# ShamG1/marl-traffic-intersection

Measured on AMD Instinct MI355X. Metric: agent-steps/sec (whole node) at 4096 envs × 8 agents × 64-beam lidar; 1/2/4/8 GPU, higher is better.
Workload: dtype f32

## Files before the change

marl-traffic-intersection_amd/csrc/mev_kernels.hip:

```cpp
#include <type_traits>

#include <cfloat>
#include <cstdlib>

#include "mev_kernels.h"
#include "mev_world.h"
#include "mev_nsort.h"

namespace mev {

#ifdef MEV_STAMPS
#define STAMP_RAW(k)                                                     \
    do {                                                                 \
        __builtin_amdgcn_wave_barrier();                                 \
        if (threadIdx.x == 0) p.debug[e * 8 + (k)] = __builtin_amdgcn_s_memtime(); \
    } while (0)
#if defined(MEV_STAMPS_R)
#undef STAMP_RAW
#define STAMP_RAW(k)                                                     \
    do {                                                                 \
        __builtin_amdgcn_wave_barrier();                                 \
        if (threadIdx.x == 0) p.debug[e * 8 + (k)] = __builtin_amdgcn_s_memrealtime(); \
    } while (0)
#ifndef MEV_STAMPS_POSTEND
#define MEV_STAMPS_POSTEND 0
#endif
#define STAMP(k) do { if ((k) == 0) STAMP_RAW(1); if ((k) == (MEV_STAMPS_POSTEND ? 6 : 5)) STAMP_RAW(2); } while (0)
#else
#define STAMP(k) STAMP_RAW(k)
#endif
#elif defined(MEV_STAMPS_Q)
__shared__ unsigned long long mev_qst[8 * 8];
#define QSTAMP(k) do { if ((threadIdx.x & 63) == 0) mev_qst[(threadIdx.x >> 6) * 8 + (k)] = __builtin_amdgcn_s_memtime(); } while (0)
#define STAMP(k) do { if ((k) == 0) QSTAMP(1); if ((k) == 1) QSTAMP(2); if ((k) == 2) QSTAMP(3); \
                      if ((k) == 5) QSTAMP(4); if ((k) == 6) QSTAMP(6); } while (0)
#else
#define STAMP(k) do {} while (0)
#endif
#ifndef QSTAMP
#define QSTAMP(k) do {} while (0)
// ... 2352 lines not shown
                const size_t g = (size_t)z * en + (size_t)e * N + tid;
                if (a.rows.reward) gmem(a.rows.reward)[g] = 0.0f;
                if (a.rows.done) gmem(a.rows.done)[g] = 0;
                if (a.rows.status) gmem(a.rows.status)[g] = 0;
                if constexpr (SAMPLE) {
                    if (sc.in->actions_out) (void)sample_action(sc, N, e, tid, z, true);
                }
            }
        }
        if constexpr (EVAL) {
            if (bad) {
                const EvalOuts& ev = a.ev;
                if (tid < N && ev.returns) gmem(ev.returns)[(size_t)e * N + tid] = 0.0f;
                if (tid == 0) {
                    if (ev.substeps) gmem(ev.substeps)[e] = 0;
                    if (ev.term) gmem(ev.term)[e] = 0;
                    if (ev.trunc) gmem(ev.trunc)[e] = 0;
                }
                if constexpr (LEAF) {
                    const Outputs& out = a.out;
                    const int ls = a.p.lidar_slots;
                    if (tid < N) gmem(a.lf.alive)[(size_t)(e - a.lf.c0) * N + tid] = 0;
                    for (int i = 0; i < N; ++i) {
                        float* row = out.obs + ((size_t)e * N + i) * out.obs_ld;
                        for (int cc = tid; cc < out.obs_ld - ls; cc += WAVE) row[cc < OBS_HEAD ? cc : cc + ls] = 0.0f;
                    }
                }
            }
        }
    }
}


template <class T>
__device__ __forceinline__ T lidar_keep(T v) {
    asm volatile("" : "+v"(v));
    return v;
}
__device__ __forceinline__ int safe_steps(float safe, float stp, float inv_stp) {
    const int j = lidar_keep((int)(safe * inv_stp));
    return (safe >= stp) ? j : 0;
}

__device__ inline float road_safe(float fx, float fy, float dx, float dy, float idx, float idy, float iadx,
                                  float iady, float rwm, float ccen, float crf) {
    const float big = 1.0e6f;
    const float rx = fx - 375.0f, ry = fy - 375.0f;
    const float ax = fabs_f(rx), ay = fabs_f(ry);
    const float sx = ax < rwm ? rwm * iadx - rx * idx : 0.0f;
    const float sy = ay < rwm ? rwm * iady - ry * idy : 0.0f;
    const float sqm = ccen - 1.55f, rg = crf + 2.0f;
    const float qx = rx != 0.0f ? rx : dx, qy = ry != 0.0f ? ry : dy;
    const float ocx = rx - (qx >= 0.0f ? ccen : -ccen), ocy = ry - (qy >= 0.0f ? ccen : -ccen);
    const float bq = ocx * dx + ocy * dy;
    const float cq = ocx * ocx + ocy * ocy - rg * rg;
    const float disc = bq * bq - cq;
    const float troot = lidar_keep(-bq - __builtin_amdgcn_sqrtf(disc));
    const float tdisc = cq <= 0.0f ? 0.0f : ((disc < 0.0f || bq >= 0.0f) ? big : troot);
    const float tsq = fminf(sqm * iadx - rx * idx, sqm * iady - ry * idy);
    const float tq = fminf(rx * dx < 0.0f ? -rx * idx : big, ry * dy < 0.0f ? -ry * idy : big);
    const float sc = fmaxf(ax, ay) < sqm ? fminf(tdisc, fminf(tsq, tq)) : 0.0f;
    const float road = fmaxf(fmaxf(sx, sy), sc);
    const float tx = (dx > 0.0f ? 748.5f - fx : fx - 0.5f) * iadx;
    const float ty = (dy > 0.0f ? 748.5f - fy : fy - 0.5f) * iady;
    return fminf(road, fminf(tx, ty));
}

__device__ inline float road_safe_uniform(float fx, float fy, float dx, float dy, float idx, float idy, float iadx,
                                          float iady, float rwm, float ccen, float crf) {
    const float big = 1.0e6f;
    const float rx = fx - 375.0f, ry = fy - 375.0f;
    const float ax = fabs_f(rx), ay = fabs_f(ry);
    const float sqm = ccen - 1.55f, rg = crf + 2.0f;
    float road = 0.0f;
    if (__builtin_amdgcn_readfirstlane((int)(ax < rwm))) road = fmaxf(road, rwm * iadx - rx * idx);
    if (__builtin_amdgcn_readfirstlane((int)(ay < rwm))) road = fmaxf(road, rwm * iady - ry * idy);
    if (__builtin_amdgcn_readfirstlane((int)(fmaxf(ax, ay) < sqm))) {
        const float qx = rx != 0.0f ? rx : dx, qy = ry != 0.0f ? ry : dy;
        const float ocx = rx - (qx >= 0.0f ? ccen : -ccen), ocy = ry - (qy >= 0.0f ? ccen : -ccen);
        const float bq = ocx * dx + ocy * dy;
        const float cq = ocx * ocx + ocy * ocy - rg * rg;
        const float disc = bq * bq - cq;
        const float troot = lidar_keep(-bq - __builtin_amdgcn_sqrtf(disc));
        const float tdisc = cq <= 0.0f ? 0.0f : ((disc < 0.0f || bq >= 0.0f) ? big : troot);
        const float tsq = fminf(sqm * iadx - rx * idx, sqm * iady - ry * idy);
        const float tq = fminf(rx * dx < 0.0f ? -rx * idx : big, ry * dy < 0.0f ? -ry * idy : big);
        road = fmaxf(road, fminf(tdisc, fminf(tsq, tq)));
    }
    const float tx = (dx > 0.0f ? 748.5f - fx : fx - 0.5f) * iadx;
    const float ty = (dy > 0.0f ? 748.5f - fy : fy - 0.5f) * iady;
    return fminf(road, fminf(tx, ty));
}

__device__ inline float atan2_fast(float y, float x) {
    const float ax = fabs_f(x), ay = fabs_f(y);
    const float mx = fmaxf(ax, ay), mn = fminf(ax, ay);
    const float t = mn * __builtin_amdgcn_rcpf(fmaxf(mx, 1e-30f));
    const float s2 = t * t;
    float r = ((-0.0464964749f * s2 + 0.15931422f) * s2 - 0.327622764f) * s2 * t + t;
    r = ay > ax ? 1.57079637f - r : r;
    r = x < 0.0f ? 3.14159274f - r : r;
    return y < 0.0f ? -r : r;
}

__device__ inline float wrap_pi_fast(float a) { return a - 6.28318531f * rintf(a * 0.159154943f); }

__device__ inline float box_lo(int lo) { return (float)(lo > 0 ? lo : lo - 1) - 0.01f; }
__device__ inline float box_hi(int hi) { return (float)hi + 1.01f; }

__device__ inline void slab_clip(float c0, float dc, float idc, float a, float b, float& lo, float& hi) {
    if (fabs_f(dc) < 1e-6f) {
        if (c0 < a || c0 > b) { lo = 1.0f; hi = 0.0f; }
        return;
    }
    const float t1 = (a - c0) * idc, t2 = (b - c0) * idc;
    lo = fmaxf(lo, fminf(t1, t2));
    hi = fminf(hi, fmaxf(t1, t2));
}




#ifndef MEV_LIDAR_NPR
#define MEV_LIDAR_NPR 2
#endif
constexpr int LIDAR_NPR = MEV_LIDAR_NPR;
constexpr int kMarchHelp = 16;
constexpr int kNptHelp = 3;
static_assert(kMarchHelp <= 32, "helper groups have at least 2 lanes");

int lidar_group(int R) {
    int g = 256 / (R > 0 ? R : 1);
    return g < 1 ? 1 : (g > 64 ? 64 : g);
}

struct LidarSrcHbm {
    static constexpr bool kBoxLds = false;
    const SimParams& p;
    __device__ float rel(int b) const { return gmem(p.rel_angles)[b]; }
    __device__ bool alive(int g) const { return gmem(p.ego.alive)[g] != 0; }
    __device__ float4 pose(int g) const { return make_float4(egof(p, EF_X)[g], egof(p, EF_Y)[g], egof(p, EF_H)[g], __int_as_float(g)); }
    __device__ void cand(int g, unsigned long long& c0, unsigned long long& c1) const {
        c0 = gmem(p.ob_cand)[2 * g];
        c1 = gmem(p.ob_cand)[2 * g + 1];
    }
    __device__ int4 box(int g, int o) const { return p.ob_box[(size_t)(g / p.N) * p.ob_stride + o]; }
};
struct LidarSrcLds {
    static constexpr bool kBoxLds = true;
    const CarsLDS& el;
    int g0;
    __device__ float rel(int b) const { return el.rel[b]; }
    __device__ bool alive(int g) const { return el.alive[g - g0] != 0; }
    __device__ float4 pose(int g) const {
        const int i = g - g0;
        return make_float4(el.x[i], el.y[i], el.h[i], __int_as_float(g));
    }
    __device__ void cand(int g, unsigned long long& c0, unsigned long long& c1) const {
        c0 = el.cand[2 * (g - g0)];
// ... 5 lines not shown
struct LidarSrcLdsEnvs {
    static constexpr bool kBoxLds = true;
    const CarsLDS& el0;
    int reg;
    const float* relp;
    int env[ENVS];
    __device__ int off(int g) const {
        int j = 0;
#pragma unroll
        for (int u = 1; u < ENVS; ++u) j = g == env[u] ? u : j;
        return j * reg;
    }
    template <class T>
    __device__ const T* at(const T* p0, int g) const {
        return reinterpret_cast<const T*>(reinterpret_cast<const unsigned char*>(p0) + off(g));
    }
    __device__ float rel(int b) const { return relp[b]; }
    __device__ bool alive(int g) const { return at(el0.alive, g)[0] != 0; }
    __device__ float4 pose(int g) const {
        return make_float4(at(el0.x, g)[0], at(el0.y, g)[0], at(el0.h, g)[0], __int_as_float(g));
    }
    __device__ void cand(int g, unsigned long long& c0, unsigned long long& c1) const {
        const unsigned long long* c = at(el0.cand, g);
        c0 = c[0];
        c1 = c[1];
    }
    __device__ int4 box(int g, int o) const { return at(el0.box, g)[o]; }
};

#ifndef MEV_DENSE_ILP
#define MEV_DENSE_ILP 2
#endif
template <bool TAB, int ILP, class Src, int NPT = LIDAR_NPR, bool HELP = false, int PART = 0, int P1 = 0,
          bool WC = false, bool SEGL = false>
__device__ __forceinline__ void lidar_body(const SimParams& p, const Outputs& out, const Src& src, const int G,
                                           const int a0, const int na, const int lane, unsigned char* base,
                                           const LidarLayout& lay, const unsigned long long redo = 0ull,
                                           const unsigned long long alive_in = 0ull) {
    static_assert(!WC || (!TAB && P1 >= WAVE), "the reference's world: no distance table, the beams at compile time");
    using W = StepWorld<WC>;
    using RW = StepRows<WC, P1>;
    const int R = P1 >= WAVE ? P1 : p.R;
    const int LS = P1 >= WAVE ? P1 : p.lidar_slots;
    float4* ag = reinterpret_cast<float4*>(base + lay.ag);
    float2* dir = reinterpret_cast<float2*>(base + lay.dir);
    int* res = reinterpret_cast<int*>(base + lay.res);
#if defined(MEV_STAMPS_R)
    const int se_ = a0 / p.N, sp_ = ((a0 % p.N) / G) & 1;
    if (lane == 0) p.debug[se_ * 8 + 3 + sp_] = __builtin_amdgcn_s_memrealtime();
#endif

    bool alv = false;
    if (PART != 0) alv = (alive_in >> lane) & 1ull;
    else if (lane < na) alv = src.alive(a0 + lane);
    const unsigned long long am = PART != 0 ? alive_in : ballot(alv);
    const int nal = __popcll(am);
    if (PART == 0 && alv) {
        const int g = a0 + lane;
        ag[lane_rank(am)] = src.pose(g);
    }
    if (PART != 2 && __popcll(am) != na) {
        for (int j = 0; j < na; ++j) {
            if ((am >> j) & 1ull) continue;
            if (RW::lidar_u8(out)) {
                uint8_t* crow = RW::lidar_u8(out) + (size_t)(a0 + j) * LS;
                for (int b = lane; b < LS; b += WAVE) crow[b] = (uint8_t)kLidarCodeDead;
                continue;
// ... 29 lines not shown
    auto probes_n = [&](auto np, float cx_, float cy_, float dx_, float dy_, int k_, float& fx, float& fy) -> int {
        int r = -1;
#pragma unroll
        for (int t = 0; t < decltype(np)::value; ++t) {
            const int c = probe(cx_, cy_, dx_, dy_, k_ + t, fx, fy);
            r = r >= 0 ? r : c;
        }
        return r;
    };
    auto probes = [&](float cx_, float cy_, float dx_, float dy_, int k_, float& fx, float& fy) -> int {
        return probes_n(std::integral_constant<int, LIDAR_NPR>{}, cx_, cy_, dx_, dy_, k_, fx, fy);
    };

    unsigned short* queue = reinterpret_cast<unsigned short*>(base + lay.queue);
    int qn = 0;
    const float rel_c0 = lane < R ? src.rel(lane) : 0.0f;
    const float rel_c1 = lane + WAVE < R ? src.rel(lane + WAVE) : 0.0f;
    auto setup = [&](const float4& a, float rel_b, auto small, float2& d, bool uni) -> int {
        float sn, cs;
#if defined(MEV_EXP_FASTSIN)
        sn = __sinf(a.z + rel_b);
        cs = __cosf(a.z + rel_b);
        (void)small;
#else
        if constexpr (decltype(small)::value) sincosf_below120(a.z + rel_b, &sn, &cs);
        else sincosf(a.z + rel_b, &sn, &cs);
#endif
        const float dx = cs, dy = -sn;
        d = make_float2(dx, dy);
        const int px = (int)a.x, py = (int)a.y;
        const unsigned pmax = (unsigned)px > (unsigned)py ? (unsigned)px : (unsigned)py;
        const float idx = __builtin_amdgcn_rcpf(dx), idy = __builtin_amdgcn_rcpf(dy);
        float safe;
        if (uni)
            safe = road_safe_uniform(a.x, a.y, dx, dy, idx, idy, fabs_f(idx), fabs_f(idy), rwm, ccen, crf);
        else
            safe = road_safe(a.x, a.y, dx, dy, idx, idy, fabs_f(idx), fabs_f(idy), rwm, ccen, crf);
        const int k1 = pmax < (unsigned)WIDTH ? 1 + safe_steps(safe, stp, inv_stp) : 0;
        float fx, fy;
        const int r = probes_n(std::integral_constant<int, LIDAR_NPR>{}, a.x, a.y, dx, dy, k1, fx, fy);
        return r >= 0 ? r : -(k1 + LIDAR_NPR) - 1;
    };
    auto pass1_one = [&](auto small, const int j) {
        const float4 a = ag[j];
        for (int b0 = 0; b0 < R; b0 += WAVE) {
            const int b = b0 + lane;
            const bool vb = b < R;
            const float rel_b = b0 == 0 ? rel_c0 : (b0 == WAVE ? rel_c1 : (vb ? src.rel(b) : 0.0f));
            float2 d;
            const int r = setup(a, rel_b, small, d, true);
            if (vb) {
                dir[j * R + b] = d;
                res[j * R + b] = r >= 0 ? r : -r - 1;
            }
            const bool pend = vb && r < 0;
            const unsigned long long m = ballot(pend);
            if (pend) queue[qn + lane_rank(m)] = (unsigned short)(j * R + b);
            qn += __popcll(m);
        }
    };
    const bool dense = P1 >= WAVE ? (P1 & (WAVE - 1)) != 0 : (P1 == 2 || (P1 == 0 && (R & (WAVE - 1)) != 0 && nal > 1));
    auto phase1 = [&](auto small) {
        if constexpr (PART == 2) {
            for (unsigned long long tm = redo; tm; tm &= tm - 1ull) pass1_one(small, __builtin_ctzll(tm));
        } else if (dense) {
            const float invRp = 1.0f / (float)R;
            const int nq = nal * R;
// ... 48 lines not shown
                    if (vb && in) {
                        dir[(j + u) * R + b] = d[u];
                        res[(j + u) * R + b] = r[u] >= 0 ? r[u] : -r[u] - 1;
                    }
                    const bool pend = vb && in && r[u] < 0;
                    const unsigned long long m = ballot(pend);
                    if (pend) queue[qn + lane_rank(m)] = (unsigned short)((j + u) * R + b);
                    qn += __popcll(m);
                }
            }
        }
        }
    };
    const bool hsmall = ballot(lane < nal && !(fabs_f(ag[lane < nal ? lane : 0].z) < 100.0f)) == 0ull;
    if (ILP > 1 && hsmall) phase1(std::true_type{});
    else phase1(std::false_type{});
    wave_lds_sync();
#if defined(MEV_EXP_STOP) && MEV_EXP_STOP == 2
    if (Src::kBoxLds) return;
#endif
#if defined(MEV_STAMPS_R)
    if (lane == 0 && na == p.N) p.debug[se_ * 8 + 4] = __builtin_amdgcn_s_memrealtime();
#endif

    if (PART == 0) __builtin_amdgcn_s_setprio(kPrioP2);
#if defined(MEV_EXP_TSNOMARCH)
    if constexpr (PART == 1) return;
#endif
    const float invR = 1.0f / (float)R;
    int next = qn < WAVE ? qn : WAVE;
    int slot = lane < qn ? (int)queue[lane] : -1;
    float cx = 0.0f, cy = 0.0f, dx = 0.0f, dy = 0.0f, idx = 0.0f, idy = 0.0f, iadx = 0.0f, iady = 0.0f;
    int k = 0;
    auto load_beam = [&](int qq) {
        const int j = (int)(((float)qq + 0.5f) * invR);
        const float4 a = ag[j];
        const float2 d = dir[qq];
        cx = a.x; cy = a.y; dx = d.x; dy = d.y;
        idx = __builtin_amdgcn_rcpf(dx);
        idy = __builtin_amdgcn_rcpf(dy);
        iadx = fabs_f(idx);
        iady = fabs_f(idy);
        k = res[qq];
    };
    if (slot >= 0) load_beam(slot);
    int* hscr = reinterpret_cast<int*>(base + lay.scr);
    bool help = false;
    while (ballot(slot >= 0) != 0ull) {
        if (HELP && next >= qn && __popcll(ballot(slot >= 0)) <= kMarchHelp) {
            help = true;
            break;
        }
        const bool act = slot >= 0;
        float fx, fy;
        int r, npr = LIDAR_NPR;
        if (NPT != LIDAR_NPR && next >= qn) {
            r = probes_n(std::integral_constant<int, NPT>{}, cx, cy, dx, dy, k, fx, fy);
            npr = NPT;
        } else {
            r = probes(cx, cy, dx, dy, k, fx, fy);
        }
        const float safe = road_safe(fx, fy, dx, dy, idx, idy, iadx, iady, rwm, ccen, crf);
        const int kn = k + npr + safe_steps(safe, stp, inv_stp);
        const bool fin = act & ((r >= 0) | (kn >= S));
        if (fin) res[slot] = r >= 0 ? r : (S << 1);
        k = kn;
        const unsigned long long fm = ballot(fin);
        if (fm != 0ull) {
            if (fin) {
                const int nq = next + lane_rank(fm);
                slot = nq < qn ? (int)queue[nq] : -1;
                if (slot >= 0) load_beam(slot);
            }
            next += __popcll(fm);
        }
    }
    if (HELP && help) {
        constexpr int NPH = kNptHelp;
        const unsigned long long am = ballot(slot >= 0);
        const int nb = __popcll(am);
        if (slot >= 0) {
            const int rk = lane_rank(am);
            hscr[2 * rk] = slot;
            hscr[2 * rk + 1] = k;
        }
        wave_lds_sync();
        auto group_march = [&](auto gs_c) {
            constexpr int GS = decltype(gs_c)::value;
            const int gi = lane / GS, j = lane & (GS - 1);
            slot = gi < nb ? hscr[2 * gi] : -1;
            const int k_h = gi < nb ? hscr[2 * gi + 1] : 0;
            if (slot >= 0) load_beam(slot);
            k = k_h;
            while (ballot(slot >= 0) != 0ull) {
                float fx, fy;
                const int k0 = k + j * NPH;
                int r = probes_n(std::integral_constant<int, NPH>{}, cx, cy, dx, dy, k0, fx, fy);
                r = r >= 0 ? r : 0x7fffffff;
                const float safe = road_safe(fx, fy, dx, dy, idx, idy, iadx, iady, rwm, ccen, crf);
                int kn = k0 + NPH + safe_steps(safe, stp, inv_stp);
                r = min(r, __builtin_amdgcn_mov_dpp(r, 0xB1, 0xf, 0xf, false));
                if constexpr (GS == 2) {
                    kn = __builtin_amdgcn_mov_dpp(kn, 0xF5, 0xf, 0xf, false);
                } else {
                    r = min(r, __builtin_amdgcn_mov_dpp(r, 0x4E, 0xf, 0xf, false));
                    kn = __builtin_amdgcn_mov_dpp(kn, 0xFF, 0xf, 0xf, false);
                    if constexpr (GS == 8) {
                        r = min(r, __builtin_amdgcn_mov_dpp(r, 0x141, 0xf, 0xf, false));
                        const int km = __builtin_amdgcn_mov_dpp(kn, 0x141, 0xf, 0xf, false);
                        kn = j < 4 ? km : kn;
                    }
                }
                const bool fin = slot >= 0 && (r != 0x7fffffff || kn >= S);
                if (fin && j == 0) res[slot] = r != 0x7fffffff ? r : (S << 1);
                slot = fin ? -1 : slot;
                k = kn;
            }
        };
        if (nb <= 8) group_march(std::integral_constant<int, 8>{});
        else if (nb <= 16) group_march(std::integral_constant<int, 4>{});
        else group_march(std::integral_constant<int, 2>{});
    }
    wave_lds_sync();
    if constexpr (PART == 1) return;
#if defined(MEV_EXP_STOP) && MEV_EXP_STOP == 3
    if (Src::kBoxLds) return;
#endif
#if defined(MEV_STAMPS_R)
    if (lane == 0 && na == p.N) p.debug[se_ * 8 + 6] = __builtin_amdgcn_s_memrealtime();
#endif

    __builtin_amdgcn_s_setprio(kPrioP3);
    int* seg_jo = reinterpret_cast<int*>(base + lay.seg_jo);
    int4* seg_rg = reinterpret_cast<int4*>(base + lay.seg_rg);
    int4* seg_bx = reinterpret_cast<int4*>(base + lay.seg_bx);
    int* scr = reinterpret_cast<int*>(base + lay.scr);
    int M = 0;
#if defined(MEV_SEG_COUNTS)
    int dbg_t = 0, dbg_pass = 0;
#endif
    if constexpr (!SEGL) {
    unsigned long long cl0 = 0ull, cl1 = 0ull;
    if (lane < nal) src.cand(__float_as_int(ag[lane].w), cl0, cl1);
    for (int j = 0; j < nal; ++j) {
        const unsigned long long c0 = readlane64(cl0, j), c1 = readlane64(cl1, j);
        const int n0 = __popcll(c0);
        if ((c0 >> lane) & 1ull) seg_jo[M + lane_rank(c0)] = (j << 8) | lane;
        if ((c1 >> lane) & 1ull) seg_jo[M + n0 + lane_rank(c1)] = (j << 8) | (lane + WAVE);
        M += n0 + __popcll(c1);
    }
    wave_lds_sync();
    }
    const float rel0 = src.rel(0);
    const bool all_beams = R == 1 || !W::beam_cull(p);
    const float dphi = R > 1 ? (src.rel(R - 1) - rel0) / (float)(R - 1) : 1.0f;
// ... 261 lines not shown
            int rr[8];
#pragma unroll
            for (int u = 0; u < 8; ++u) rr[u] = (j0 + u < nal && beam) ? res[(j0 + u) * R + lane] : 0;
#pragma unroll
            for (int u = 0; u < 8; ++u) {
                if (j0 + u < nal && beam) {
                    const int g = __builtin_amdgcn_readlane(gl, j0 + u);
                    obs_store<true>(&out.obs[(size_t)g * RW::obs_ld(out) + OBS_HEAD + lane], row_value(rr[u]));
                }
            }
        }
    } else {
        for (int j = 0; j < nal; ++j) {
            const int g = __float_as_int(ag[j].w);
            float* row = out.obs + (size_t)g * RW::obs_ld(out) + OBS_HEAD;
            for (int b = lane; b < LS; b += WAVE)
                obs_store<true>(row + b, ((res[j * R + b] & 1) ? march_dist<TAB, WC>(p, res[j * R + b] >> 1) : W::lidar_max(p)) *
                                             W::lidar_inv(p));
        }
    }
}

template <bool TAB>
__global__ __launch_bounds__(256, 8) void k_lidar(SimParams p, Outputs out, int G, int a_begin, int a_end) {
    extern __shared__ __align__(16) unsigned char lds_raw[];
    const int lane = threadIdx.x & (WAVE - 1);
    const int wv = threadIdx.x / WAVE;
    const int blk = xcd_env((int)blockIdx.x, (int)gridDim.x);
    const int a0 = __builtin_amdgcn_readfirstlane(a_begin + (blk * (int)(blockDim.x / WAVE) + wv) * G);
    if (a0 >= a_end) return;
    const int na = a_end - a0 < G ? a_end - a0 : G;
    __builtin_amdgcn_s_setprio(kPrioLidar);
    const LidarLayout lay = lidar_layout(G, p.R, lidar_cand_max(p));
    lidar_body<TAB, 1>(p, out, LidarSrcHbm{p}, G, a0, na, lane, lds_raw + (size_t)wv * (size_t)lay.bytes, lay);
}


template <int NM, int KM>
__host__ __device__ inline StepLayout step_layout_t(const SimParams& p) {
    if constexpr (NM == 0) return step_layout(p);
    else return StepLayout{FixedLayout<NM, KM>::rel, FixedLayout<NM, KM>::rel, FixedLayout<NM, KM>::envw,
                           FixedLayout<NM, KM>::lidar, FixedLayout<NM, KM>::bytes};
}
#ifndef MEV_PHASE1_ILP
#define MEV_PHASE1_ILP 2
#endif
#ifndef MEV_ESPLIT_ILP
#define MEV_ESPLIT_ILP 1
#endif
constexpr int kPhase1Ilp = MEV_PHASE1_ILP;
constexpr int kEsplitIlp = MEV_ESPLIT_ILP;

template <bool TRAFFIC>
__device__ __forceinline__ void deal_append(const SimParams& p, const StepInputs& in, const CarsCtx& cx, const int e) {
    if constexpr (TRAFFIC) {
        if (!(in.deal & 2)) return;
        const int lane0 = threadIdx.x & (WAVE - 1);
        const int x = (int)blockIdx.x & (kDealLists - 1);
        const int nxt = in.deal_ring == 2 ? 0 : in.deal_ring + 1;
        if (lane0 == 0) {
            const int c = (in.auto_reset && cx.ended) ? 0 : (cx.ncnt < kDealClasses - 1 ? cx.ncnt : kDealClasses - 1);
            const int slot = atomicAdd(p.deal_cnt + (size_t)nxt * kDealRingInts + (x * kDealClasses + c) * kDealPad, 1);
            const size_t ring_off = (size_t)nxt * kDealLists * kDealClasses * (size_t)p.E;
            gmem(p.deal_order)[ring_off + ((size_t)x * kDealClasses + c) * p.E + slot] = e;
        }
        if (blockIdx.x == 0 && lane0 < kDealLists * kDealClasses) {
            const int clr = nxt == 2 ? 0 : nxt + 1;
// ... 650 lines not shown
```

marl-traffic-intersection_amd/csrc/mev_step_body.inc:

```
    static_assert(!SPLIT || !TRAFFIC || ESPLIT, "split waves with traffic: the early split");
    static_assert(!WC || (!TRAFFIC && !TAB && NM > 0 && PK == 1 && !SPLIT && P1 >= WAVE && NC > 0),
                  "the world at compile time: one wave per env, the counts at compile time, no table");
    const SimParams& p = *pp;
    extern __shared__ __align__(16) unsigned char step_lds[];
    const int wv = SPLIT ? __builtin_amdgcn_readfirstlane((int)(threadIdx.x >> 6)) : 0;
    int npc_cls = kDealClasses - 1;
    const int e = (TRAFFIC && (in.deal & 1)) ? deal_env(p, in.deal_ring, (int)blockIdx.x, 1, 0, &npc_cls)
                                             : xcd_env((int)blockIdx.x, (int)gridDim.x) * PK;
#if defined(MEV_STAMPS_R)
    STAMP_RAW(0);
#endif
    QSTAMP(0);
    constexpr int KF = TRAFFIC ? KM : 0;
    constexpr bool SEGL = NM == 8 && KF == 0;
    constexpr int NCE = NM == 1 ? 1 : NC;
    const StepLayout sl = step_layout_t<NM, KF>(p);
    constexpr bool DIMS = NM == 0;
    using NLT = NpcLDST<KM, DIMS>;
    CarsLDS el = NM ? carve_cars_lds(step_lds, NM, KF) : carve_cars_lds(step_lds, p.N, cars_k(p), DIMS);
    el.head = reinterpret_cast<float*>(step_lds + sl.head);
    el.rel = reinterpret_cast<float*>(step_lds + sl.rel);
    el.envw = reinterpret_cast<int32_t*>(step_lds + sl.envw);
    if constexpr (!TRAFFIC && NM > 0) {
        static_assert(NM == 0 || FixedLayout<(NM ? NM : 1), 0>::lay.bytes >= kWinBytes, "LDS path windows");
// ... 33 lines not shown
#pragma unroll
        for (int j = 0; j < PK; ++j)
            es[j] = (in.deal & 1) ? deal_env(p, in.deal_ring, b, PK, j) : xcd_env(b, (int)gridDim.x) * PK + j;
        unsigned char* lbase = step_lds + PK * REG;
        constexpr LidarLayout lay = lidar_layout_beams(PK, PK * kTsplitRays, KF, false);
        float* rel0 = reinterpret_cast<float*>(step_lds + sl.rel);
        for (int bb = lane; bb < p.R; bb += WAVE) rel0[bb] = gmem(p.rel_angles)[bb];
        const unsigned long long am = ts_ego_phase<PK, KF>(p, in, step_lds, REG, es, lane);
        const bool on = lane < PK;
        const bool alive = ((am >> lane) & 1ull) != 0;
        int ee = es[0];
#pragma unroll
        for (int j = 1; j < PK; ++j) ee = lane == j ? es[j] : ee;
        for (unsigned long long dm = ballot(on && !alive); dm; dm &= dm - 1ull) {
            const int g = __builtin_amdgcn_readlane(ee, __builtin_ctzll(dm));
            if (out.lidar_u8) {
                for (int bb = lane; bb < p.lidar_slots; bb += WAVE)
                    out.lidar_u8[(size_t)g * p.lidar_slots + bb] = (uint8_t)kLidarCodeDead;
            } else {
                for (int bb = lane; bb < p.lidar_slots; bb += WAVE) out.obs[(size_t)g * out.obs_ld + OBS_HEAD + bb] = 0.0f;
            }
        }
        float4* ag = reinterpret_cast<float4*>(lbase + lay.ag);
        if (alive) {
            const CarsLDS elp = carve_cars_lds(step_lds + lane * REG, 1, KF);
            ag[lane_rank(am)] = make_float4(elp.x[0], elp.y[0], elp.h[0], __int_as_float(ee));
        }
        wave_lds_sync();
        const CarsLDS el0 = carve_cars_lds(step_lds, 1, KF);
        LidarSrcLdsEnvs<PK> src{el0, REG, rel0, {}};
#pragma unroll
        for (int j = 0; j < PK; ++j) src.env[j] = es[j];
        const int nal = __popcll(am);
        lidar_body<TAB, kEsplitIlp, LidarSrcLdsEnvs<PK>, LIDAR_NPR, true, 1, P1>(p, out, src, PK, 0, nal, lane, lbase,
                                                                             lay, 0ull, am);
        __syncthreads();
        __syncthreads();
        const int li = on ? lane : 0;
        const bool rs = alive && (reinterpret_cast<const int32_t*>(step_lds + li * REG + sl.envw)[6] & 1) != 0;
        const unsigned long long rl = ballot(rs);
        unsigned long long redo = 0ull;
        if (rl != 0ull) {
            if (rs) {
                const CarsLDS elr = carve_cars_lds(step_lds + li * REG, 1, KF);
                ag[lane_rank(am)] = make_float4(elr.x[0], elr.y[0], elr.h[0], __int_as_float(ee));
            }
            for (unsigned long long m = rl; m; m &= m - 1ull) {
                const int i = __builtin_ctzll(m);
                redo |= 1ull << __popcll(am & ((1ull << i) - 1ull));
            }
            wave_lds_sync();
        }
        __builtin_amdgcn_s_setprio(kPrioEsplitCarPhase);
        lidar_body<TAB, kEsplitIlp, LidarSrcLdsEnvs<PK>, LIDAR_NPR, true, 2, P1>(p, out, src, PK, 0, nal, lane, lbase,
                                                                             lay, redo, am);
        return;
    } else if constexpr (ESPLIT) {
        static_assert(SPLIT && !TRAFFIC && NM > 0, "early split without traffic: two waves");
        const int lane = threadIdx.x & (WAVE - 1);
        const int NE = NCE ? NCE : p.N;
        const int g0 = e * NE;
        const int NS = PK == 1 ? NE : (p.E - e < PK ? p.E - e : PK) * NE;
        unsigned char* lbase = step_lds + sl.lidar;
        const LidarLayout lay = FixedLayout<(NM ? NM : 1), 0>::lay;
        if (wv == 0) {
            __builtin_amdgcn_s_setprio(kPrioEsplitCars);
            CarsCtx cx = cars_pre<false, true, NLT, PK, false, true, false, false, NCE>(p, in, out, e, el, nl);
            cars_post<false, true, NLT, PK, false, NCE>(p, out, e, el, nl, cx);
        } else {
            __builtin_amdgcn_s_setprio(kPrioEsplitRoad);
            for (int b = lane; b < p.R; b += WAVE) el.rel[b] = gmem(p.rel_angles)[b];
            const bool on = lane < NS;
            const int il = on ? lane : 0;
            const int ee = PK == 1 ? e : e + il / NE;
            const uint32_t ug = (uint32_t)(g0 + il);
            const bool pend = ldu(gmem(p.pending_reset), (uint32_t)ee) != 0;
            const int route_l = ldu(egoi(p, EF_ROUTE), ug);
            Kin k{ldu(egof(p, EF_X), ug), ldu(egof(p, EF_Y), ug), ldu(egof(p, EF_V), ug), ldu(egof(p, EF_H), ug),
                  ldu(egof(p, EF_ACC), ug), ldu(egof(p, EF_STEER), ug)};
            bool alive = ldu(gmem(p.ego.alive), ug) != 0;
            const float a0 = ldu(gmem(in.actions), 2 * ug), a1 = ldu(gmem(in.actions), 2 * ug + 1);
            if (in.auto_reset && pend) {
                const int rid = reset_route(p, in.rng_counter, ee, PK == 1 ? il : il - (ee - e) * NE, route_l);
                k = Kin{gmem(p.rt.spawn)[3 * rid], gmem(p.rt.spawn)[3 * rid + 1], 0.0f, gmem(p.rt.spawn)[3 * rid + 2],
                        0.0f, 0.0f};
                alive = true;
            }
            {
                Kin ku = k;
                float sH, cH;
                car_update_heading(ku, a0, a1, in.dt);
                sincosf(alive ? ku.h : k.h, &sH, &cH);
                car_update_move(ku, cH, sH);
                if (alive) k = ku;
            }
            alive = on && alive;
            const unsigned long long am = ballot(alive);
            float4* ag = reinterpret_cast<float4*>(lbase + lay.ag);
            if (alive) ag[lane_rank(am)] = make_float4(k.x, k.y, k.h, __int_as_float(g0 + il));
            wave_lds_sync();
            lidar_body<TAB, kEsplitIlp, LidarSrcLds, LIDAR_NPR, true, 1, P1, false, SEGL>(
                p, out, LidarSrcLds{el, g0}, NS, g0, NS, lane, lbase, lay, 0ull, am);
            __syncthreads();
            const unsigned rmask = (unsigned)el.envw[6];
            const bool rs = alive && lane < 32 && ((rmask >> (lane & 31)) & 1u);
            const unsigned long long rl = ballot(rs);
            unsigned long long redo = 0ull;
            if (rl != 0ull) {
                if (rs) ag[lane_rank(am)] = make_float4(el.x[lane], el.y[lane], el.h[lane], __int_as_float(g0 + lane));
                for (unsigned long long m = rl; m; m &= m - 1ull) {
                    const int i = __builtin_ctzll(m);
                    redo |= 1ull << __popcll(am & ((1ull << i) - 1ull));
                }
                wave_lds_sync();
            }
            __builtin_amdgcn_s_setprio(kPrioEsplitCarPhase);
            lidar_body<TAB, kEsplitIlp, LidarSrcLds, LIDAR_NPR, true, 2, P1, false, SEGL>(
                p, out, LidarSrcLds{el, g0}, NS, g0, NS, lane, lbase, lay, redo, am);
        }
        return;
    }
    if constexpr (!(TRAFFIC && ESPLIT)) {
    CarsCtx cx{};
    if (wv == 0) cx = cars_pre<TRAFFIC, true, NLT, PK, (!TRAFFIC && NM > 0), false, DIMS, false, NCE, false, WC>(p, in, out, e, el, nl, npc_cls);
    if (SPLIT) __syncthreads();
    else wave_lds_sync();
#if !defined(MEV_EXP_STOP) || MEV_EXP_STOP != 0
    if (wv == 0) {
        cars_post<TRAFFIC, true, NLT, PK, DIMS, NCE, false, (WC ? P1 : 0)>(p, out, e, el, nl, cx);
        wave_lds_sync();
    }
#endif
    deal_append<TRAFFIC>(p, in, cx, e);
#if defined(MEV_EXP_STOP) && MEV_EXP_STOP == 0
    return;
#endif
    if (SPLIT && wv == 0) return;
#if defined(MEV_EXP_STOP) && MEV_EXP_STOP == 1
    return;
#endif
    const int NEC = NCE ? NCE : p.N;
    const int NS = PK == 1 ? NEC : (p.E - e < PK ? p.E - e : PK) * NEC;
    int G = 512 / (p.R > 0 ? p.R : 1);
    G = G < 1 ? 1 : (G < NS ? G : NS);
    if (PK == 1) G = (NCE > 0 && P1 >= WAVE) ? step_pool_n(NCE, P1) : step_pool(p);
    const LidarLayout lay = NM ? FixedLayout<(NM ? NM : 1), KF>::lay : lidar_layout(G, p.R, lidar_cand_max(p), false);
    unsigned char* lbase = step_lds + sl.lidar;
    const int lane = threadIdx.x & (WAVE - 1);
    const int g0 = e * NEC;
    for (int j0 = 0; j0 < NS; j0 += G) {
        if (j0 > 0) wave_lds_sync();
        if (j0 > 0) __builtin_amdgcn_s_setprio(kPrioLidar);
        const int na = NS - j0 < G ? NS - j0 : G;
        lidar_body<TAB, kPhase1Ilp, LidarSrcLds, LIDAR_NPR, true, 0, P1, WC, SEGL>(
            p, out, LidarSrcLds{el, g0}, G, g0 + j0, na, lane, lbase, lay);
    }
#if defined(MEV_STAMPS_Q)
    QSTAMP(7);
    if ((threadIdx.x & 63) == 0)
        for (int q = 0; q < 8; ++q) p.debug[e * 8 + q] = mev_qst[wv * 8 + q];
#endif
#if defined(MEV_STAMPS_R)
    if (!SPLIT || wv == 1) {
        const unsigned long long t = __builtin_amdgcn_s_memrealtime() & ((1ull << 40) - 1);
        const unsigned hw = __builtin_amdgcn_s_getreg((15 << 11) | 4) & 0xffffu;
        const unsigned xcc = __builtin_amdgcn_s_getreg((3 << 11) | 20) & 7u;
        if (lane == 0) p.debug[e * 8 + 7] = t | ((unsigned long long)(hw | (xcc << 16)) << 40);
    }
#endif
    }
```

Before: 1.260 billion.

## Add road-entry safe-distance bound for lidar march and early group exit

Adds a new analytic bound, road_entry_safe, that computes how far a lidar ray can travel before it can enter road-boundary geometry. The goal is larger safe skips during the march and fewer probe iterations. It is enabled by default only for the non-traffic step lidar paths. The group-march loop now does its hit reduction before the bound computation and exits early once every active group has a hit, skipping further bound evaluation. It also moves the road_safe helpers into a shared header and adds optional iteration-count instrumentation. The risk is that any mismatch between the new bound and the exact road check could change lidar outputs.

```diff
diff --git a/marl-traffic-intersection_amd/csrc/mev_kernels.hip b/marl-traffic-intersection_amd/csrc/mev_kernels.hip
--- a/marl-traffic-intersection_amd/csrc/mev_kernels.hip
+++ b/marl-traffic-intersection_amd/csrc/mev_kernels.hip
@@ -6,6 +6,7 @@
 #include "mev_kernels.h"
 #include "mev_world.h"
 #include "mev_nsort.h"
+#include "mev_roadbound.h"
 
 namespace mev {
 
@@ -2424,65 +2425,11 @@
 }
 
 
-template <class T>
-__device__ __forceinline__ T lidar_keep(T v) {
-    asm volatile("" : "+v"(v));
-    return v;
-}
 __device__ __forceinline__ int safe_steps(float safe, float stp, float inv_stp) {
     const int j = lidar_keep((int)(safe * inv_stp));
     return (safe >= stp) ? j : 0;
 }
 
-__device__ inline float road_safe(float fx, float fy, float dx, float dy, float idx, float idy, float iadx,
-                                  float iady, float rwm, float ccen, float crf) {
-    const float big = 1.0e6f;
-    const float rx = fx - 375.0f, ry = fy - 375.0f;
-    const float ax = fabs_f(rx), ay = fabs_f(ry);
-    const float sx = ax < rwm ? rwm * iadx - rx * idx : 0.0f;
-    const float sy = ay < rwm ? rwm * iady - ry * idy : 0.0f;
-    const float sqm = ccen - 1.55f, rg = crf + 2.0f;
-    const float qx = rx != 0.0f ? rx : dx, qy = ry != 0.0f ? ry : dy;
-    const float ocx = rx - (qx >= 0.0f ? ccen : -ccen), ocy = ry - (qy >= 0.0f ? ccen : -ccen);
-    const float bq = ocx * dx + ocy * dy;
-    const float cq = ocx * ocx + ocy * ocy - rg * rg;
-    const float disc = bq * bq - cq;
-    const float troot = lidar_keep(-bq - __builtin_amdgcn_sqrtf(disc));
-    const float tdisc = cq <= 0.0f ? 0.0f : ((disc < 0.0f || bq >= 0.0f) ? big : troot);
-    const float tsq = fminf(sqm * iadx - rx * idx, sqm * iady - ry * idy);
-    const float tq = fminf(rx * dx < 0.0f ? -rx * idx : big, ry * dy < 0.0f ? -ry * idy : big);
-    const float sc = fmaxf(ax, ay) < sqm ? fminf(tdisc, fminf(tsq, tq)) : 0.0f;
-    const float road = fmaxf(fmaxf(sx, sy), sc);
-    const float tx = (dx > 0.0f ? 748.5f - fx : fx - 0.5f) * iadx;
-    const float ty = (dy > 0.0f ? 748.5f - fy : fy - 0.5f) * iady;
-    return fminf(road, fminf(tx, ty));
-}
-
-__device__ inline float road_safe_uniform(float fx, float fy, float dx, float dy, float idx, float idy, float iadx,
-                                          float iady, float rwm, float ccen, float crf) {
-    const float big = 1.0e6f;
-    const float rx = fx - 375.0f, ry = fy - 375.0f;
-    const float ax = fabs_f(rx), ay = fabs_f(ry);
-    const float sqm = ccen - 1.55f, rg = crf + 2.0f;
-    float road = 0.0f;
-    if (__builtin_amdgcn_readfirstlane((int)(ax < rwm))) road = fmaxf(road, rwm * iadx - rx * idx);
-    if (__builtin_amdgcn_readfirstlane((int)(ay < rwm))) road = fmaxf(road, rwm * iady - ry * idy);
-    if (__builtin_amdgcn_readfirstlane((int)(fmaxf(ax, ay) < sqm))) {
-        const float qx = rx != 0.0f ? rx : dx, qy = ry != 0.0f ? ry : dy;
-        const float ocx = rx - (qx >= 0.0f ? ccen : -ccen), ocy = ry - (qy >= 0.0f ? ccen : -ccen);
-        const float bq = ocx * dx + ocy * dy;
-        const float cq = ocx * ocx + ocy * ocy - rg * rg;
-        const float disc = bq * bq - cq;
-        const float troot = lidar_keep(-bq - __builtin_amdgcn_sqrtf(disc));
-        const float tdisc = cq <= 0.0f ? 0.0f : ((disc < 0.0f || bq >= 0.0f) ? big : troot);
-        const float tsq = fminf(sqm * iadx - rx * idx, sqm * iady - ry * idy);
-        const float tq = fminf(rx * dx < 0.0f ? -rx * idx : big, ry * dy < 0.0f ? -ry * idy : big);
-        road = fmaxf(road, fminf(tdisc, fminf(tsq, tq)));
-    }
-    const float tx = (dx > 0.0f ? 748.5f - fx : fx - 0.5f) * iadx;
-    const float ty = (dy > 0.0f ? 748.5f - fy : fy - 0.5f) * iady;
-    return fminf(road, fminf(tx, ty));
-}
 
 __device__ inline float atan2_fast(float y, float x) {
     const float ax = fabs_f(x), ay = fabs_f(y);
@@ -2517,6 +2464,11 @@
 #define MEV_LIDAR_NPR 2
 #endif
 constexpr int LIDAR_NPR = MEV_LIDAR_NPR;
+#if defined(MEV_ROAD_BOUND)
+constexpr int kRoadBoundStep = MEV_ROAD_BOUND, kRoadBoundTraffic = MEV_ROAD_BOUND, kRoadBoundLidar = MEV_ROAD_BOUND;
+#else
+constexpr int kRoadBoundStep = 1, kRoadBoundTraffic = 0, kRoadBoundLidar = 0;
+#endif
 constexpr int kMarchHelp = 16;
 constexpr int kNptHelp = 3;
 static_assert(kMarchHelp <= 32, "helper groups have at least 2 lanes");
@@ -2588,7 +2540,7 @@
 #define MEV_DENSE_ILP 2
 #endif
 template <bool TAB, int ILP, class Src, int NPT = LIDAR_NPR, bool HELP = false, int PART = 0, int P1 = 0,
-          bool WC = false, bool SEGL = false>
+          bool WC = false, bool SEGL = false, int RB = 0>
 __device__ __forceinline__ void lidar_body(const SimParams& p, const Outputs& out, const Src& src, const int G,
                                            const int a0, const int na, const int lane, unsigned char* base,
                                            const LidarLayout& lay, const unsigned long long redo = 0ull,
@@ -2684,7 +2636,9 @@
         const unsigned pmax = (unsigned)px > (unsigned)py ? (unsigned)px : (unsigned)py;
         const float idx = __builtin_amdgcn_rcpf(dx), idy = __builtin_amdgcn_rcpf(dy);
         float safe;
-        if (uni)
+        if constexpr (RB == 1)
+            safe = road_entry_safe(a.x, a.y, dx, dy, idx, idy, fabs_f(idx), fabs_f(idy), rwm, ccen, crf);
+        else if (uni)
             safe = road_safe_uniform(a.x, a.y, dx, dy, idx, idy, fabs_f(idx), fabs_f(idy), rwm, ccen, crf);
         else
             safe = road_safe(a.x, a.y, dx, dy, idx, idy, fabs_f(idx), fabs_f(idy), rwm, ccen, crf);
@@ -2799,6 +2753,10 @@
     int slot = lane < qn ? (int)queue[lane] : -1;
     float cx = 0.0f, cy = 0.0f, dx = 0.0f, dy = 0.0f, idx = 0.0f, idy = 0.0f, iadx = 0.0f, iady = 0.0f;
     int k = 0;
+    auto bound2 = [&](float fx, float fy) -> float {
+        if constexpr (RB == 1) return road_entry_safe(fx, fy, dx, dy, idx, idy, iadx, iady, rwm, ccen, crf);
+        else return road_safe(fx, fy, dx, dy, idx, idy, iadx, iady, rwm, ccen, crf);
+    };
     auto load_beam = [&](int qq) {
         const int j = (int)(((float)qq + 0.5f) * invR);
         const float4 a = ag[j];
@@ -2813,12 +2771,19 @@
     if (slot >= 0) load_beam(slot);
     int* hscr = reinterpret_cast<int*>(base + lay.scr);
     bool help = false;
+#if defined(MEV_ITER_COUNTS)
+    int ic_pool = 0, ic_grp = 0, ic_busy = 0, ic_nb = 0;
+#endif
     while (ballot(slot >= 0) != 0ull) {
         if (HELP && next >= qn && __popcll(ballot(slot >= 0)) <= kMarchHelp) {
             help = true;
             break;
         }
         const bool act = slot >= 0;
+#if defined(MEV_ITER_COUNTS)
+        ++ic_pool;
+        ic_busy += __popcll(ballot(act));
+#endif
         float fx, fy;
         int r, npr = LIDAR_NPR;
         if (NPT != LIDAR_NPR && next >= qn) {
@@ -2827,8 +2792,7 @@
         } else {
             r = probes(cx, cy, dx, dy, k, fx, fy);
         }
-        const float safe = road_safe(fx, fy, dx, dy, idx, idy, iadx, iady, rwm, ccen, crf);
-        const int kn = k + npr + safe_steps(safe, stp, inv_stp);
+        const int kn = k + npr + safe_steps(bound2(fx, fy), stp, inv_stp);
         const bool fin = act & ((r >= 0) | (kn >= S));
         if (fin) res[slot] = r >= 0 ? r : (S << 1);
         k = kn;
@@ -2846,6 +2810,9 @@
         constexpr int NPH = kNptHelp;
         const unsigned long long am = ballot(slot >= 0);
         const int nb = __popcll(am);
+#if defined(MEV_ITER_COUNTS)
+        ic_nb = nb;
+#endif
         if (slot >= 0) {
             const int rk = lane_rank(am);
             hscr[2 * rk] = slot;
@@ -2860,20 +2827,31 @@
             if (slot >= 0) load_beam(slot);
             k = k_h;
             while (ballot(slot >= 0) != 0ull) {
+#if defined(MEV_ITER_COUNTS)
+                ++ic_grp;
+                ic_busy += __popcll(ballot(slot >= 0));
+#endif
                 float fx, fy;
                 const int k0 = k + j * NPH;
                 int r = probes_n(std::integral_constant<int, NPH>{}, cx, cy, dx, dy, k0, fx, fy);
                 r = r >= 0 ? r : 0x7fffffff;
-                const float safe = road_safe(fx, fy, dx, dy, idx, idy, iadx, iady, rwm, ccen, crf);
-                int kn = k0 + NPH + safe_steps(safe, stp, inv_stp);
                 r = min(r, __builtin_amdgcn_mov_dpp(r, 0xB1, 0xf, 0xf, false));
+                if constexpr (GS != 2) {
+                    r = min(r, __builtin_amdgcn_mov_dpp(r, 0x4E, 0xf, 0xf, false));
+                    if constexpr (GS == 8) r = min(r, __builtin_amdgcn_mov_dpp(r, 0x141, 0xf, 0xf, false));
+                }
+                if constexpr (RB == 1) {
+                    if (ballot(slot >= 0 && r == 0x7fffffff) == 0ull) {
+                        if (slot >= 0 && j == 0) res[slot] = r;
+                        break;
+                    }
+                }
+                int kn = k0 + NPH + safe_steps(bound2(fx, fy), stp, inv_stp);
                 if constexpr (GS == 2) {
                     kn = __builtin_amdgcn_mov_dpp(kn, 0xF5, 0xf, 0xf, false);
                 } else {
-                    r = min(r, __builtin_amdgcn_mov_dpp(r, 0x4E, 0xf, 0xf, false));
                     kn = __builtin_amdgcn_mov_dpp(kn, 0xFF, 0xf, 0xf, false);
                     if constexpr (GS == 8) {
-                        r = min(r, __builtin_amdgcn_mov_dpp(r, 0x141, 0xf, 0xf, false));
                         const int km = __builtin_amdgcn_mov_dpp(kn, 0x141, 0xf, 0xf, false);
                         kn = j < 4 ? km : kn;
                     }
@@ -2888,6 +2866,16 @@
         else if (nb <= 16) group_march(std::integral_constant<int, 4>{});
         else group_march(std::integral_constant<int, 2>{});
     }
+#if defined(MEV_ITER_COUNTS)
+    if (lane == 0 && na == p.N) {
+        unsigned long long* dbg = p.debug + (size_t)(a0 / p.N) * 8;
+        dbg[0] = (unsigned long long)(ic_pool + ic_grp);
+        dbg[1] = (unsigned long long)qn;
+        dbg[2] = (unsigned long long)ic_pool;
+        dbg[3] = (unsigned long long)ic_busy;
+        dbg[4] = (unsigned long long)ic_nb;
+    }
+#endif
     wave_lds_sync();
     if constexpr (PART == 1) return;
 #if defined(MEV_EXP_STOP) && MEV_EXP_STOP == 3
@@ -3215,7 +3203,7 @@
     const int na = a_end - a0 < G ? a_end - a0 : G;
     __builtin_amdgcn_s_setprio(kPrioLidar);
     const LidarLayout lay = lidar_layout(G, p.R, lidar_cand_max(p));
-    lidar_body<TAB, 1>(p, out, LidarSrcHbm{p}, G, a0, na, lane, lds_raw + (size_t)wv * (size_t)lay.bytes, lay);
+    lidar_body<TAB, 1, LidarSrcHbm, LIDAR_NPR, false, 0, 0, false, false, kRoadBoundLidar>(p, out, LidarSrcHbm{p}, G, a0, na, lane, lds_raw + (size_t)wv * (size_t)lay.bytes, lay);
 }
 
 
diff --git a/marl-traffic-intersection_amd/csrc/mev_roadbound.h b/marl-traffic-intersection_amd/csrc/mev_roadbound.h
--- /dev/null
+++ b/marl-traffic-intersection_amd/csrc/mev_roadbound.h
@@ -0,0 +1,118 @@
+#pragma once
+
+#include "mev_math.h"
+
+namespace mev {
+
+template <class T>
+MEV_HD T lidar_keep(T v) {
+#if defined(__HIP_DEVICE_COMPILE__)
+    asm volatile("" : "+v"(v));
+#endif
+    return v;
+}
+MEV_HD float rb_sqrt(float x) {
+#if defined(__HIP_DEVICE_COMPILE__)
+    return __builtin_amdgcn_sqrtf(x);
+#else
+    return __builtin_sqrtf(x);
+#endif
+}
+MEV_HD bool rb_uniform(bool c) {
+#if defined(__HIP_DEVICE_COMPILE__)
+    return __builtin_amdgcn_readfirstlane((int)c) != 0;
+#else
+    return c;
+#endif
+}
+MEV_HD float rb_min(float a, float b) { return __builtin_fminf(a, b); }
+MEV_HD float rb_max(float a, float b) { return __builtin_fmaxf(a, b); }
+
+MEV_HD float road_safe(float fx, float fy, float dx, float dy, float idx, float idy, float iadx, float iady, float rwm,
+                       float ccen, float crf) {
+    const float big = 1.0e6f;
+    const float rx = fx - 375.0f, ry = fy - 375.0f;
+    const float ax = fabs_f(rx), ay = fabs_f(ry);
+    const float sx = ax < rwm ? rwm * iadx - rx * idx : 0.0f;
+    const float sy = ay < rwm ? rwm * iady - ry * idy : 0.0f;
+    const float sqm = ccen - 1.55f, rg = crf + 2.0f;
+    const float qx = rx != 0.0f ? rx : dx, qy = ry != 0.0f ? ry : dy;
+    const float ocx = rx - (qx >= 0.0f ? ccen : -ccen), ocy = ry - (qy >= 0.0f ? ccen : -ccen);
+    const float bq = ocx * dx + ocy * dy;
+    const float cq = ocx * ocx + ocy * ocy - rg * rg;
+    const float disc = bq * bq - cq;
+    const float troot = lidar_keep(-bq - rb_sqrt(disc));
+    const float tdisc = cq <= 0.0f ? 0.0f : ((disc < 0.0f || bq >= 0.0f) ? big : troot);
+    const float tsq = rb_min(sqm * iadx - rx * idx, sqm * iady - ry * idy);
+    const float tq = rb_min(rx * dx < 0.0f ? -rx * idx : big, ry * dy < 0.0f ? -ry * idy : big);
+    const float sc = rb_max(ax, ay) < sqm ? rb_min(tdisc, rb_min(tsq, tq)) : 0.0f;
+    const float road = rb_max(rb_max(sx, sy), sc);
+    const float tx = (dx > 0.0f ? 748.5f - fx : fx - 0.5f) * iadx;
+    const float ty = (dy > 0.0f ? 748.5f - fy : fy - 0.5f) * iady;
+    return rb_min(road, rb_min(tx, ty));
+}
+
+MEV_HD float road_safe_uniform(float fx, float fy, float dx, float dy, float idx, float idy, float iadx, float iady,
+                               float rwm, float ccen, float crf) {
+    const float big = 1.0e6f;
+    const float rx = fx - 375.0f, ry = fy - 375.0f;
+    const float ax = fabs_f(rx), ay = fabs_f(ry);
+    const float sqm = ccen - 1.55f, rg = crf + 2.0f;
+    float road = 0.0f;
+    if (rb_uniform(ax < rwm)) road = rb_max(road, rwm * iadx - rx * idx);
+    if (rb_uniform(ay < rwm)) road = rb_max(road, rwm * iady - ry * idy);
+    if (rb_uniform(rb_max(ax, ay) < sqm)) {
+        const float qx = rx != 0.0f ? rx : dx, qy = ry != 0.0f ? ry : dy;
+        const float ocx = rx - (qx >= 0.0f ? ccen : -ccen), ocy = ry - (qy >= 0.0f ? ccen : -ccen);
+        const float bq = ocx * dx + ocy * dy;
+        const float cq = ocx * ocx + ocy * ocy - rg * rg;
+        const float disc = bq * bq - cq;
+        const float troot = lidar_keep(-bq - rb_sqrt(disc));
+        const float tdisc = cq <= 0.0f ? 0.0f : ((disc < 0.0f || bq >= 0.0f) ? big : troot);
+        const float tsq = rb_min(sqm * iadx - rx * idx, sqm * iady - ry * idy);
+        const float tq = rb_min(rx * dx < 0.0f ? -rx * idx : big, ry * dy < 0.0f ? -ry * idy : big);
+        road = rb_max(road, rb_min(tdisc, rb_min(tsq, tq)));
+    }
+    const float tx = (dx > 0.0f ? 748.5f - fx : fx - 0.5f) * iadx;
+    const float ty = (dy > 0.0f ? 748.5f - fy : fy - 0.5f) * iady;
+    return rb_min(road, rb_min(tx, ty));
+}
+
+MEV_HD float road_entry_safe(float fx, float fy, float dx, float dy, float idx, float idy, float iadx, float iady,
+                             float rwm, float ccen, float crf) {
+    (void)idx;
+    (void)idy;
+    const float never = 1.0e6f;
+    const float rx = fx - 375.0f, ry = fy - 375.0f;
+    const float sqm = ccen - 1.55f, rg = crf + 2.0f;
+    const float x = dx < 0.0f ? -rx : rx, y = dy < 0.0f ? -ry : ry;
+    const float a = fabs_f(dx), b = fabs_f(dy);
+    const float txp = (rwm - x) * iadx, txm = (-rwm - x) * iadx, txs = (sqm - x) * iadx;
+    const float typ = (rwm - y) * iady, tym = (-rwm - y) * iady, tys = (sqm - y) * iady;
+    const float inx = rb_max(txp, 0.0f), iny = rb_max(typ, 0.0f);
+    const float t1 = rb_max(inx, iny);
+    const bool xn = x < -rwm, yn = y < -rwm;
+    const bool v4 = xn && yn;
+    const bool v2 = xn && iny < txm;
+    const bool v3 = yn && inx < tym;
+    const float mA = v2 ? iny : (v3 ? inx : t1);
+    const float oA = v2 ? txm : (v3 ? tym : never);
+    const float mB = (v2 || v3) ? t1 : never;
+    const float m1 = v4 ? 0.0f : mA, o1 = v4 ? rb_min(txm, tym) : oA, m2 = v4 ? mA : mB;
+    const bool xg = !(v4 || v2), yg = !(v4 || v3);
+    const float ue = fabs_f(x + a * m1), ve = fabs_f(y + b * m1);
+    const float ocx = ue - ccen, ocy = ve - ccen;
+    const float bq = ocx * (xg ? a : -a) + ocy * (yg ? b : -b);
+    const float cq = ocx * ocx + ocy * ocy - rg * rg;
+    const float disc = bq * bq - cq;
+    const float troot = lidar_keep(-bq - rb_sqrt(disc));
+    const float tdisc = cq <= 0.0f ? 0.0f : ((disc < 0.0f || bq >= 0.0f) ? never : troot);
+    const float tcorner = rb_min(m1 + tdisc, rb_min(xg ? txs : never, yg ? tys : never));
+    const float tq = rb_max(ue, ve) >= sqm ? m1 : (tcorner < o1 ? tcorner : never);
+    const float road = rb_min(tq, m2);
+    const float tx = ((dx > 0.0f ? 373.5f : 374.5f) - x) * iadx;
+    const float ty = ((dy > 0.0f ? 373.5f : 374.5f) - y) * iady;
+    return rb_min(road, rb_min(tx, ty));
+}
+
+}
diff --git a/marl-traffic-intersection_amd/csrc/mev_step_body.inc b/marl-traffic-intersection_amd/csrc/mev_step_body.inc
--- a/marl-traffic-intersection_amd/csrc/mev_step_body.inc
+++ b/marl-traffic-intersection_amd/csrc/mev_step_body.inc
@@ -89,8 +89,8 @@
 #pragma unroll
         for (int j = 0; j < PK; ++j) src.env[j] = es[j];
         const int nal = __popcll(am);
-        lidar_body<TAB, kEsplitIlp, LidarSrcLdsEnvs<PK>, LIDAR_NPR, true, 1, P1>(p, out, src, PK, 0, nal, lane, lbase,
-                                                                             lay, 0ull, am);
+        lidar_body<TAB, kEsplitIlp, LidarSrcLdsEnvs<PK>, LIDAR_NPR, true, 1, P1, false, false, kRoadBoundTraffic>(
+            p, out, src, PK, 0, nal, lane, lbase, lay, 0ull, am);
         __syncthreads();
         __syncthreads();
         const int li = on ? lane : 0;
@@ -109,8 +109,8 @@
             wave_lds_sync();
         }
         __builtin_amdgcn_s_setprio(kPrioEsplitCarPhase);
-        lidar_body<TAB, kEsplitIlp, LidarSrcLdsEnvs<PK>, LIDAR_NPR, true, 2, P1>(p, out, src, PK, 0, nal, lane, lbase,
-                                                                             lay, redo, am);
+        lidar_body<TAB, kEsplitIlp, LidarSrcLdsEnvs<PK>, LIDAR_NPR, true, 2, P1, false, false, kRoadBoundTraffic>(
+            p, out, src, PK, 0, nal, lane, lbase, lay, redo, am);
         return;
     } else if constexpr (ESPLIT) {
         static_assert(SPLIT && !TRAFFIC && NM > 0, "early split without traffic: two waves");
@@ -156,7 +156,7 @@
             float4* ag = reinterpret_cast<float4*>(lbase + lay.ag);
             if (alive) ag[lane_rank(am)] = make_float4(k.x, k.y, k.h, __int_as_float(g0 + il));
             wave_lds_sync();
-            lidar_body<TAB, kEsplitIlp, LidarSrcLds, LIDAR_NPR, true, 1, P1, false, SEGL>(
+            lidar_body<TAB, kEsplitIlp, LidarSrcLds, LIDAR_NPR, true, 1, P1, false, SEGL, kRoadBoundStep>(
                 p, out, LidarSrcLds{el, g0}, NS, g0, NS, lane, lbase, lay, 0ull, am);
             __syncthreads();
             const unsigned rmask = (unsigned)el.envw[6];
@@ -172,7 +172,7 @@
                 wave_lds_sync();
             }
             __builtin_amdgcn_s_setprio(kPrioEsplitCarPhase);
-            lidar_body<TAB, kEsplitIlp, LidarSrcLds, LIDAR_NPR, true, 2, P1, false, SEGL>(
+            lidar_body<TAB, kEsplitIlp, LidarSrcLds, LIDAR_NPR, true, 2, P1, false, SEGL, kRoadBoundStep>(
                 p, out, LidarSrcLds{el, g0}, NS, g0, NS, lane, lbase, lay, redo, am);
         }
         return;
@@ -209,7 +209,8 @@
         if (j0 > 0) wave_lds_sync();
         if (j0 > 0) __builtin_amdgcn_s_setprio(kPrioLidar);
         const int na = NS - j0 < G ? NS - j0 : G;
-        lidar_body<TAB, kPhase1Ilp, LidarSrcLds, LIDAR_NPR, true, 0, P1, WC, SEGL>(
+        lidar_body<TAB, kPhase1Ilp, LidarSrcLds, LIDAR_NPR, true, 0, P1, WC, SEGL,
+                   (TRAFFIC ? kRoadBoundTraffic : kRoadBoundStep)>(
             p, out, LidarSrcLds{el, g0}, G, g0 + j0, na, lane, lbase, lay);
     }
 #if defined(MEV_STAMPS_Q)
```

Measured after the change: 1.275 billion, median of 6. 1.2% higher.
